# pola-rs/polars

Measured on NVIDIA H100. Metric: group_by_agg_rows_per_sec, higher is better.
Workload: dtype int64/float64

## Files before the change

### polars_b200/csrc/groupby.cu

```cuda
#include <algorithm>
#include <cmath>
#include <cstdio>
#include <cstdlib>

#include "common.cuh"
#include "dev_utils.cuh"
#include "groupby.h"
#include "groupby_dev.cuh"

namespace plb {

__device__ __forceinline__ uint64_t make_policy_evict_last() {
    uint64_t p; asm volatile("createpolicy.fractional.L2::evict_last.b64 %0, 1.0;" : "=l"(p)); return p;
}
__device__ __forceinline__ uint64_t tbl_load(const uint64_t* p, uint64_t pol, int hint) {
    uint64_t v;
    if (hint & 2) asm volatile("ld.global.ca.u64 %0, [%1];" : "=l"(v) : "l"(p) : "memory");
    else if (hint & 1) asm volatile("ld.global.cg.L2::cache_hint.u64 %0, [%1], %2;" : "=l"(v) : "l"(p), "l"(pol));
    else v = __ldcg(reinterpret_cast<const unsigned long long*>(p));
    return v;
}

__device__ __forceinline__ uint64_t* gb_resolve(const GbTableDev& T, uint64_t key, uint64_t slot, uint64_t k, uint64_t pol, int hint) {
    const uint64_t mask = T.cap - 1;
// ... 316 lines not shown
            __syncwarp();
        }
#pragma unroll
        for (int r = 0; r < 2; r++) {
            if (kind[r] < 0 || hidx[r] >= 0) continue;
            uint64_t* e = kind[r] == 0 ? gb_resolve(T, key[r], slot[r], k0[r], 0, khint) : gb_special(T, kind[r] - 1);
            if (e) gb_apply_row<MAXC>(L, T, B, e, 2 * p + r, [&](int c) { return raw[c][r]; });
        }
    }
    gb_tail_row(L, T, B);
    __syncwarp();
    for (int h = lane; h < H.rows; h += 32) {
        const uint64_t* arow = wacc + h * row_words;
        if ((uint32_t)arow[1] == 0) continue;
        gb_merge_row(L, T, arow, h == H.n_hot ? 1 : (h == H.n_hot + 1 ? 2 : 0));
    }
}

__global__ void k_gb_init(uint64_t* entries, int64_t n_entries, int stride, int soa, int pw, const __grid_constant__ GbLayout L) {
    const int64_t total = n_entries * stride;
    for (int64_t i = (int64_t)blockIdx.x * blockDim.x + threadIdx.x; i < total; i += (int64_t)gridDim.x * blockDim.x) {
        int w = soa ? (int)(i / n_entries) : (int)(i % stride);
        if (pw) {
            if (w == 1 || w == 2) w = ((i - n_entries) & 1) ? pw : 1;
            else if (w == pw) w = 2;
        }
        uint64_t v = 0;
        if (w == 0) v = GB_EMPTY; else if (w == 1) v = GB_W1_INIT; else if (w - 2 < L.n_words) v = L.init[w - 2];
        entries[i] = v;
    }
}

constexpr int GB_CAND_MAX = 1024;
struct GbSampleStats { unsigned distinct, f1, f2, adjacent, nulls, empties, n_cand, pad; };
struct GbCandidate { uint64_t key; uint64_t mult; };
__global__ void k_gb_estimate(const void* keys, const uint32_t* key_validity, int key_dtype, int64_t n, int64_t m, uint64_t* scratch, unsigned* mult, uint64_t cap, int shift, GbSampleStats* stats) {
    for (int64_t i = (int64_t)blockIdx.x * blockDim.x + threadIdx.x; i < m; i += (int64_t)gridDim.x * blockDim.x) {
        int64_t row = (int64_t)(((unsigned __int128)i * (unsigned __int128)n) / (unsigned __int128)m);
        bool ins = false, adj = false, isnull = false, isempty = false;
        if (key_validity == nullptr || bit_get(key_validity, row)) {
            uint64_t key = load_key_rt(keys, key_dtype, row);
            adj = row + 1 < n && load_key_rt(keys, key_dtype, row + 1) == key && (key_validity == nullptr || bit_get(key_validity, row + 1));
            if (key != GB_EMPTY) {
                uint64_t slot = table_hash(key) >> shift;
                for (int pr = 0; pr < (int)cap; pr++) {
                    uint64_t k = __ldcg(reinterpret_cast<const unsigned long long*>(scratch + slot));
                    if (k == GB_EMPTY) {
                        unsigned long long old = atomicCAS(reinterpret_cast<unsigned long long*>(scratch + slot), (unsigned long long)GB_EMPTY, (unsigned long long)key);
                        if (old == GB_EMPTY) { ins = true; k = key; } else k = old;
                    }
                    if (k == key) { atomicAdd(mult + slot, 1u); break; }
                    slot = (slot + 1) & (cap - 1);
                }
            } else isempty = true;
        } else {
            isnull = true;
            adj = row + 1 < n && !bit_get(key_validity, row + 1);
        }
        unsigned act = __activemask();
        unsigned b = __ballot_sync(act, ins), a = __ballot_sync(act, adj), bn = __ballot_sync(act, isnull), be = __ballot_sync(act, isempty);
        if (lane_id() == (unsigned)(__ffs(act) - 1)) {
            if (b) atomicAdd(&stats->distinct, (unsigned)__popc(b));
            if (a) atomicAdd(&stats->adjacent, (unsigned)__popc(a));
            if (bn) atomicAdd(&stats->nulls, (unsigned)__popc(bn));
            if (be) atomicAdd(&stats->empties, (unsigned)__popc(be));
        }
    }
}
__global__ void k_gb_estimate_stats(const uint64_t* scratch, const unsigned* mult, int64_t cap, unsigned hot_thr, GbSampleStats* stats, GbCandidate* cand) {
    unsigned f1 = 0, f2 = 0;
    for (int64_t i = (int64_t)blockIdx.x * blockDim.x + threadIdx.x; i < cap; i += (int64_t)gridDim.x * blockDim.x) {
        const unsigned c = mult[i];
        f1 += c == 1; f2 += c == 2;
        if (c >= hot_thr) {
            const unsigned at = atomicAdd(&stats->n_cand, 1u);
            if (at < GB_CAND_MAX) { cand[at].key = scratch[i]; cand[at].mult = c; }
        }
    }
    f1 = __reduce_add_sync(0xffffffffu, f1); f2 = __reduce_add_sync(0xffffffffu, f2);
    if (lane_id() == 0) { if (f1) atomicAdd(&stats->f1, f1); if (f2) atomicAdd(&stats->f2, f2); }
}
__global__ void k_fill_u64(uint64_t* p, uint64_t v, int64_t n) {
    for (int64_t i = (int64_t)blockIdx.x * blockDim.x + threadIdx.x; i < n; i += (int64_t)gridDim.x * blockDim.x) p[i] = v;
}

__device__ __forceinline__ void gb_merge_row(const GbLayout& L, const GbTableDev& T, const uint64_t* src, int meta, int64_t sws, int64_t sslot, int spw) {
    uint64_t* e = meta == 1 ? gb_special(T, 0) : (meta == 2 ? gb_special(T, 1) : gb_find_or_insert(T, src[0]));
    if (!e) return;
    const uint64_t lf = src[gb_woff(sslot, 1, sws, spw)];
    if ((uint32_t)lf) atomicAdd(reinterpret_cast<unsigned*>(gb_wp(T, e, 1)), (uint32_t)lf);
    if ((uint32_t)(lf >> 32) != 0xFFFFFFFFu) atomicMin(reinterpret_cast<unsigned*>(gb_wp(T, e, 1)) + 1, (uint32_t)(lf >> 32));
    for (int w = 0; w < L.n_words; w++) {
        const uint64_t v = src[gb_woff(sslot, 2 + w, sws, spw)];
        if (v == L.init[w]) continue;
        uint64_t* a = gb_wp(T, e, 2 + w);
        switch (L.slot_op[w]) {
            case W_ADD_F64: atomicAdd(reinterpret_cast<double*>(a), __longlong_as_double((long long)v)); break;
            case W_MIN_S64: atomicMin(reinterpret_cast<long long*>(a), (long long)v); break;
            case W_MAX_S64: atomicMax(reinterpret_cast<long long*>(a), (long long)v); break;
            case W_MIN_U64: case W_MIN_F64: atomicMin(reinterpret_cast<unsigned long long*>(a), (unsigned long long)v); break;
            case W_MAX_U64: case W_MAX_F64: atomicMax(reinterpret_cast<unsigned long long*>(a), (unsigned long long)v); break;
            default: atomicAdd(reinterpret_cast<unsigned long long*>(a), (unsigned long long)v); break;
        }
    }
}
__global__ void __launch_bounds__(256) k_gb_merge(const __grid_constant__ GbLayout L, const __grid_constant__ GbTableDev T, const uint64_t* __restrict__ rows, int64_t n_rows, int64_t src_es, int64_t src_ws, int table_mode, int64_t src_cap, int src_pw) {
    for (int64_t r = (int64_t)blockIdx.x * blockDim.x + threadIdx.x; r < n_rows; r += (int64_t)gridDim.x * blockDim.x) {
        const uint64_t* src = rows + r * src_es;
        int meta;
        if (table_mode) { if (src[0] == GB_EMPTY) continue; meta = r == src_cap ? 1 : (r == src_cap + 1 ? 2 : 0); }
        else meta = (int)src[(L.n_words + 2) * src_ws];
        gb_merge_row(L, T, src, meta, src_ws, r, table_mode ? src_pw : 0);
    }
// ... 391 lines not shown
    if (d >= m * 0.995) return n;
    double lo = d, hi = n > d ? n : d;
    for (int it = 0; it < 60; it++) { double G = 0.5 * (lo + hi); double ex = G * (1.0 - exp(-m / G)); if (ex < d) lo = G; else hi = G; }
    return hi;
}

void GroupByState::build_hot_list(const void* cand_v, int n_cand, bool null_hot, bool empty_hot, double m) {
    const GbCandidate* cand = static_cast<const GbCandidate*>(cand_v);
    hot = GbHotDev{}; hot_share = 0; hot_buf.reset();
    if (!knob_int("BL_K5_HOTKEYS", 1) || (n_cand <= 0 && !null_hot && !empty_hot)) return;
    std::vector<GbCandidate> c(cand, cand + std::max(n_cand, 0));
    std::sort(c.begin(), c.end(), [](const GbCandidate& a, const GbCandidate& b) { return a.mult > b.mult || (a.mult == b.mult && a.key < b.key); });
    const int row_words = 2 + L.n_words;
    int n_hot = std::min<int>((int)c.size(), std::min(GB_HOT_MAX, 512 / row_words - 2));
    if (n_hot < 0) n_hot = 0;
    if (!c.empty()) hot_share = (double)c[0].mult / m;
    std::vector<unsigned char> h(GB_HOT_SLOTS * 8 + GB_HOT_SLOTS, 0);
    uint64_t* hk = reinterpret_cast<uint64_t*>(h.data());
    unsigned char* hi = h.data() + GB_HOT_SLOTS * 8;
    for (int i = 0; i < GB_HOT_SLOTS; i++) hk[i] = GB_EMPTY;
    for (int i = 0; i < n_hot; i++) {
        unsigned sl = (unsigned)(table_hash(c[i].key) >> (64 - GB_HOT_BITS));
        while (hk[sl] != GB_EMPTY) sl = (sl + 1) & (GB_HOT_SLOTS - 1);
        hk[sl] = c[i].key; hi[sl] = (unsigned char)i;
    }
    hot_buf = dev_alloc(h.size());
    PLB_CUDA(cudaMemcpyAsync(hot_buf->p, h.data(), h.size(), cudaMemcpyHostToDevice, ctx().stream));
    PLB_CUDA(cudaStreamSynchronize(ctx().stream));
    hot.keys = as<uint64_t>(hot_buf); hot.idx = reinterpret_cast<const uint8_t*>(hot_buf->p) + GB_HOT_SLOTS * 8;
    hot.n_hot = n_hot; hot.null_hot = null_hot ? 1 : 0; hot.empty_hot = empty_hot ? 1 : 0; hot.rows = n_hot + 2;
}

uint64_t GroupByState::choose_cap(const DevCol& key, int64_t n_total) {
    double G, G_raw, G_upper = 0;
    if (expected_groups > 0) G = G_raw = (double)expected_groups;
    else {
        const int64_t n = key.len, m = std::min<int64_t>(n, 65536);
        const uint64_t scap = 1 << 18;
        const size_t tail_bytes = sizeof(GbSampleStats) + sizeof(GbCandidate) * GB_CAND_MAX;
        DevPtr scratch = dev_alloc(scap * 8), mult = dev_alloc(scap * 4 + tail_bytes);
        GbSampleStats* dstats = reinterpret_cast<GbSampleStats*>(as<unsigned>(mult) + scap);
        GbCandidate* dcand = reinterpret_cast<GbCandidate*>(dstats + 1);
        const double nt = (double)std::max<int64_t>(n_total, n);
        const double hot_knob = knob_double("BL_K5_HOT_ROWS", 30000.0), hot_rows = hot_knob >= 0 ? hot_knob : 30000.0;
        const unsigned hot_thr = (unsigned)std::max(12.0, std::ceil(hot_rows * (double)m / nt));
        PLB_LAUNCH("k5_fill", k_fill_u64, grid_for(scap, 256), 256, 0, as<uint64_t>(scratch), GB_EMPTY, (int64_t)scap);
        dev_memset(mult->p, 0, scap * 4 + sizeof(GbSampleStats));
        PLB_LAUNCH("k5_estimate", k_gb_estimate, grid_for(m, 256), 256, 0, key.v(), key.vm(), key.dtype, n, m, as<uint64_t>(scratch), as<unsigned>(mult), scap, 64 - 18, dstats);
        PLB_LAUNCH("k5_estimate", k_gb_estimate_stats, grid_for(scap, 256), 256, 0, as<uint64_t>(scratch), as<unsigned>(mult), (int64_t)scap, hot_thr, dstats, dcand);
        std::vector<unsigned char> hbuf(tail_bytes);
        PLB_CUDA(cudaMemcpyAsync(hbuf.data(), dstats, tail_bytes, cudaMemcpyDeviceToHost, ctx().stream));
        PLB_CUDA(cudaStreamSynchronize(ctx().stream));
        GbSampleStats st; memcpy(&st, hbuf.data(), sizeof st);
        const GbCandidate* cand = reinterpret_cast<const GbCandidate*>(hbuf.data() + sizeof(GbSampleStats));
        G_raw = estimate_groups((double)st.distinct, (double)m, nt);
        if (m < n && st.f1 > 0) {
            const double chao = (double)st.distinct + (double)st.f1 * ((double)st.f1 - 1.0) / (2.0 * ((double)st.f2 + 1.0));
            if (chao > G_raw) G_raw = chao;
            if ((double)st.distinct >= (double)m * 0.995 && st.f2 >= 16) G_raw = std::min(G_raw, 2.0 * chao);
        }
        sample_adjacent = m > 0 ? (double)st.adjacent / (double)m : 0.0;
        if (m < n && sample_adjacent > 0.5) {
            const double q = 1.0 - sample_adjacent;
            const double runs = nt * std::min(1.0, q + 3.0 * std::sqrt(q * sample_adjacent / (double)m) + 2.0 / (double)m) + 1.0;
            if (runs < G_raw) G_raw = runs;
        }
        G = G_raw * 1.25 + 64;
        if (G > nt) G = nt;
        if (G_raw > nt) G_raw = nt;
        G_upper = std::min(nt, (double)st.distinct + (double)st.f1 / (double)m * nt);
        build_hot_list(cand, (int)std::min<unsigned>(st.n_cand, GB_CAND_MAX), st.nulls >= hot_thr, st.empties >= hot_thr, (double)m);
    }
    est_groups = (int64_t)(G_raw * 1.25) + 2;
    const double lf_knob = knob_double("BL_K5_LF", 60.0) / 100.0, lf = (lf_knob > 0.05 && lf_knob < 0.95) ? lf_knob : 0.6;
    uint64_t c = pow2_at_least(G / lf);
    const double l2_budget = 0.55 * (double)ctx().l2_bytes;
    if ((double)c * L.stride * 8 > l2_budget && G_raw / ((double)c / 2) <= 0.8 && c > 1024) c >>= 1;
    while (G_upper / lf > (double)c && (double)(2 * c) * L.stride * 8 <= l2_budget) c <<= 1;
    if (getenv("BL_K5_DEBUG"))
        fprintf(stderr, "[k5] rows=%lld est_groups=%.0f upper=%.0f cap=%llu (%.1f MB) hot_keys=%d null_hot=%d empty_hot=%d hot_share=%.4f adjacent=%.3f\n", (long long)n_total, G_raw, G_upper,
                (unsigned long long)c, (double)c * L.stride * 8 / 1e6, hot.n_hot, hot.null_hot, hot.empty_hot, hot_share, sample_adjacent);
    return c;
}

template <int KEY_ELEM, int KEY_CANON, bool KEY_NULLS, int PAIRS, bool BULK>
static void launch_consume_p(const GbLayout& L, const GbTableDev& T, const GbBatch& B, int grid) {
    with_at_least<1, 2, 4, 8>(L.n_cols, [&](auto maxc) {
        constexpr int MAXC = decltype(maxc)::value, P = MAXC == 8 ? 1 : PAIRS;
        const size_t smem = BULK ? (size_t)2 * P * 256 * 16 : 0;
        PLB_LAUNCH("k5_groupby_agg", (k_gb_consume<KEY_ELEM, KEY_CANON, KEY_NULLS, MAXC, P, BULK>), grid, 256, smem, L, T, B);
    });
}
template <int KEY_ELEM, int KEY_CANON, bool KEY_NULLS>
static void launch_consume(const GbLayout& L, const GbTableDev& T, const GbBatch& B, int grid) {
    const int pairs = knob_int("BL_K5_PAIRS", 1) == 2 ? 2 : 1;
    if (T.pw && T.bulk_lanes > 0 && L.pair_k >= 0) {
        bool lean = KEY_ELEM == 8 && KEY_CANON == 0 && T.bulk_lanes == 32 && !T.hint && !L.need_first && L.need_len && L.n_cols >= 1 && L.n_cols <= 3 &&
                    knob_int("BL_K5_LEAN", 1) != 0;
        bool nulls = KEY_NULLS;
        for (int c = 0; lean && c < L.n_cols; c++) { lean = B.cols[c].elem == 8 && L.col_kbegin[c + 1] - L.col_kbegin[c] <= 2; nulls = nulls || B.cols[c].validity != nullptr; }
        if (lean) with_at_least<1, 2, 3>(L.n_cols, [&](auto nc) { with_bool(nulls, [&](auto nl) {
            PLB_LAUNCH("k5_groupby_agg", (k_gb_consume_lean<decltype(nc)::value, decltype(nl)::value>), grid, 256, (size_t)2 * 256 * 16, L, T, B);
        }); });
        else launch_consume_p<KEY_ELEM, KEY_CANON, KEY_NULLS, 1, true>(L, T, B, grid);
    }
    else if (pairs == 2) launch_consume_p<KEY_ELEM, KEY_CANON, KEY_NULLS, 2, false>(L, T, B, grid);
// ... 529 lines not shown
```

### polars_b200/csrc/groupby.h

```cpp
#pragma once
#include <cstdlib>
#include <type_traits>

#include "common.cuh"

namespace plb {

inline int knob_int(const char* name, int dflt) { const char* e = getenv(name); return e ? atoi(e) : dflt; }
inline double knob_double(const char* name, double dflt) { const char* e = getenv(name); return e ? atof(e) : dflt; }

template <int V> using IntC = std::integral_constant<int, V>;
template <class F> void with_key_form(int key_dtype, F&& f) {
    if (dtype_size(key_dtype) == 8) { if (key_dtype == BL_FLOAT64) f(IntC<8>{}, IntC<1>{}); else f(IntC<8>{}, IntC<0>{}); }
    else { if (key_dtype == BL_FLOAT32) f(IntC<4>{}, IntC<2>{}); else f(IntC<4>{}, IntC<0>{}); }
}
template <int V, int... Vs, class F> void with_at_least(int n, F&& f) {
    if constexpr (sizeof...(Vs) == 0) f(IntC<V>{});
    else if (n <= V) f(IntC<V>{});
    else with_at_least<Vs...>(n, f);
}
template <class F> void with_bool(bool b, F&& f) { if (b) f(std::true_type{}); else f(std::false_type{}); }

constexpr uint64_t GB_EMPTY = 0x8000000000000000ULL;
constexpr uint64_t GB_W1_INIT = 0xFFFFFFFF00000000ULL;
// ... 22 lines not shown
    }
    return (int64_t)w * ws;
}
struct GbBatch {
    const void* keys; const uint32_t* key_validity; int64_t n; uint32_t row_base; int32_t key_dtype;
    GbColDev cols[GB_MAX_COLS];
};


constexpr int GB_HOT_MAX = 62;
constexpr int GB_HOT_BITS = 8;
constexpr int GB_HOT_SLOTS = 1 << GB_HOT_BITS;
struct GbHotDev { const uint64_t* keys; const uint8_t* idx; int32_t n_hot, null_hot, empty_hot, rows; };

struct GbDense { DevPtr keys, first, len, words, ctl; int64_t Gb = 0; bool ready = false; };

struct AggPlan { int kind, in_dtype, out_dtype; int main, nullcnt; bool nullable; };

struct GroupByState {
    int key_dtype;
    std::vector<int> agg_kinds, agg_dtypes;
    int64_t expected_groups;
    std::vector<AggPlan> plans;
    GbLayout L;
    bool lean_shape = false;
    int pair_word = 0;
    GbTableDev T{};
    DevPtr entries, status;
    uint64_t cap = 0;
    int64_t rows_seen = 0;
    int64_t merged_rows = 0;
    int64_t est_groups = 0;
    double sample_adjacent = 0;
    GbHotDev hot{};
    double hot_share = 0;
    DevPtr hot_buf;

    GroupByState(int key_dt, const std::vector<int>& kinds, const std::vector<int>& dtypes, const std::vector<int>& nullable, int64_t expected, bool track_first);
    void consume_all(const DevCol& key, const std::vector<const DevCol*>& values);
    bool consume_radix(const DevCol& key, const std::vector<const DevCol*>& values, uint64_t planned_cap);
    GbDense dense;
    void consume_pipelined(const DevCol& key, const std::vector<const DevCol*>& values, int64_t chunk_rows, const std::vector<cudaEvent_t>& ready);
    void consume(const DevCol& key, const std::vector<const DevCol*>& values, int64_t row_base);
    void merge_partials(const uint64_t* rows, int64_t n_rows);
    void merge_partial_regions(const uint64_t* const* ptrs, const int64_t* counts, int n_regions);
    DevPtr export_partials(int n_partitions, int* row_words_out, int64_t* offsets_host);
    void export_partials_p2p(int n_ranks, int my_rank, void* const* windows, int64_t rows_per_src, int* row_words_out, int64_t* sent_rows);
    void export_partials_p2p_async(int n_ranks, int my_rank, void* const* window_halves, int64_t rows_per_src, uint64_t epoch, int* row_words_out);
    void merge_window_async(const void* own_half, int n_ranks, int64_t rows_per_src, uint64_t epoch);
    void settle();
    int read_status();
    bool defer_status = false;
    const DevCol* redo_key = nullptr; std::vector<const DevCol*> redo_values; uint64_t redo_cap = 0;
    void finish(bool maintain_order, const DevCol* key_col_for_gather, DevCol& out_key, std::vector<DevCol>& out_aggs, DevCol* out_first = nullptr);
    void reset();
    int64_t count_groups();

   private:
    void alloc_table(uint64_t new_cap);
    int smem_table_cap() const;
    bool bind_columns(const DevCol& key, const std::vector<const DevCol*>& values, int64_t row_base, int pw, int max_cols, GbBatch& B, GbLayout& Lb) const;
    void note_batch_shape(const DevCol& key, const std::vector<const DevCol*>& values);
    uint64_t choose_cap(const DevCol& key, int64_t n_total);
    void build_hot_list(const void* candidates, int n_cand, bool null_hot, bool empty_hot, double sample_rows);
    void launch_batch(const DevCol& key, const std::vector<const DevCol*>& values, int64_t row_base);
    void grow(uint64_t new_cap);
// ... 4 lines not shown
```

### polars_b200/csrc/groupby_radix.cu

```cuda
#include <algorithm>
#include <cstdlib>

#include "common.cuh"
#include "dev_utils.cuh"
#include "groupby.h"
#include "groupby_dev.cuh"

namespace plb {

constexpr int GBR_THREADS = 512;
constexpr int GBR_MAX_LOGB = 13;
constexpr int GBR_NCW = 31, GBR_NCT = GBR_NCW * 32;

struct GbRadixDev {
    uint64_t* recs;
    const unsigned long long* off;
    unsigned* cursor;
    unsigned* counts;
    int logB, roww;
    uint64_t* special;
    int* status;
};

template <int KEY_ELEM> __device__ __forceinline__ void gbr_load_pair(const void* col, int64_t r0, int64_t n, uint64_t& a, uint64_t& b) {
    a = 0; b = 0;
    if (r0 + 1 < n) gb_load_pair<KEY_ELEM>(col, r0, a, b);
    else if (r0 < n) a = KEY_ELEM == 8 ? reinterpret_cast<const uint64_t*>(col)[r0] : reinterpret_cast<const uint32_t*>(col)[r0];
}
__device__ __forceinline__ void gbr_load_pair_rt(const void* col, int elem, int64_t r0, int64_t n, uint64_t& a, uint64_t& b) {
    if (elem == 8) gbr_load_pair<8>(col, r0, n, a, b); else gbr_load_pair<4>(col, r0, n, a, b);
}

template <int KEY_ELEM, int KEY_CANON>
__global__ void __launch_bounds__(512) k_gbr_hist(const void* __restrict__ keys, int64_t n, int logB, unsigned* __restrict__ counts) {
    extern __shared__ unsigned h_s[];
    const int B = 1 << logB;
    for (int i = threadIdx.x; i < B; i += blockDim.x) h_s[i] = 0;
    __syncthreads();
    const int64_t npairs = (n + 1) >> 1;
    for (int64_t p = (int64_t)blockIdx.x * blockDim.x + threadIdx.x; p < npairs; p += (int64_t)gridDim.x * blockDim.x) {
        uint64_t k0, k1;
        gbr_load_pair<KEY_ELEM>(keys, 2 * p, n, k0, k1);
        k0 = canon_key<KEY_CANON>(k0); k1 = canon_key<KEY_CANON>(k1);
        if (k0 != GB_EMPTY) atomicAdd(&h_s[(unsigned)(table_hash(k0) >> (64 - logB))], 1u);
        if (2 * p + 1 < n && k1 != GB_EMPTY) atomicAdd(&h_s[(unsigned)(table_hash(k1) >> (64 - logB))], 1u);
    }
    __syncthreads();
    for (int i = threadIdx.x; i < B; i += blockDim.x) if (h_s[i]) atomicAdd(&counts[i], h_s[i]);
}
__global__ void __launch_bounds__(1024) k_gbr_offsets(const unsigned* __restrict__ counts, int B, unsigned long long pad_units, unsigned pad_each, unsigned align,
                                                      unsigned long long* __restrict__ off, unsigned* __restrict__ cursor) {
    __shared__ unsigned long long wsum[32];
    __shared__ unsigned long long carry_s;
    if (threadIdx.x == 0) carry_s = 0;
    __syncthreads();
    const unsigned lane = lane_id(), warp = threadIdx.x >> 5;
    for (int base = 0; base < B; base += 1024) {
        const int i = base + threadIdx.x;
        unsigned long long c = 0;
        if (i < B) { c = counts[i]; c += (c < pad_units ? c : pad_units) * pad_each; c = (c + align - 1) & ~(unsigned long long)(align - 1); cursor[i] = 0; }
        unsigned long long x = c;
        for (int o = 1; o < 32; o <<= 1) { const unsigned long long y = __shfl_up_sync(0xffffffffu, x, o); if (lane >= (unsigned)o) x += y; }
        if (lane == 31) wsum[warp] = x;
        __syncthreads();
        if (warp == 0) {
            unsigned long long s = wsum[lane], t = s;
            for (int o = 1; o < 32; o <<= 1) { const unsigned long long y = __shfl_up_sync(0xffffffffu, t, o); if (lane >= (unsigned)o) t += y; }
            wsum[lane] = t - s;
        }
        __syncthreads();
        const unsigned long long incl = carry_s + wsum[warp] + x;
        if (i < B) off[i] = incl - c;
        __syncthreads();
        if (threadIdx.x == 1023) carry_s = incl;
        __syncthreads();
    }
    if (threadIdx.x == 0) off[B] = carry_s;
}

__device__ __forceinline__ void gbr_apply_special(const GbLayout& L, const GbBatch& Bt, uint64_t* sp, const uint64_t* raw) {
    atomicAdd(reinterpret_cast<unsigned long long*>(sp), 1ull);
    for (int c = 0; c < L.n_cols; c++)
        for (int k = L.col_kbegin[c]; k < L.col_kbegin[c + 1]; k++) {
            uint64_t* a = sp + 1 + L.wslot[k];
            const int dt = Bt.cols[c].dtype;
            switch (L.wop[k]) {
                case W_ADD_INT: atomicAdd(reinterpret_cast<unsigned long long*>(a), (unsigned long long)raw_to_int(dt, raw[c])); break;
                case W_ADD_F64: atomicAdd(reinterpret_cast<double*>(a), raw_to_f64(dt, raw[c])); break;
                case W_MIN_S64: atomicMin(reinterpret_cast<long long*>(a), (long long)raw_to_int(dt, raw[c])); break;
                case W_MAX_S64: atomicMax(reinterpret_cast<long long*>(a), (long long)raw_to_int(dt, raw[c])); break;
                case W_MIN_U64: atomicMin(reinterpret_cast<unsigned long long*>(a), (unsigned long long)raw[c]); break;
                case W_MAX_U64: atomicMax(reinterpret_cast<unsigned long long*>(a), (unsigned long long)raw[c]); break;
                case W_MIN_F64: { const double f = raw_to_f64(dt, raw[c]); if (f == f) atomicMin(reinterpret_cast<unsigned long long*>(a), (unsigned long long)f64_to_ordered(f)); break; }
// ... 25 lines not shown
        uint64_t k[RPT]; unsigned pk[RPT];
#pragma unroll
        for (int j = 0; j < RPT / 2; j++) gbr_load_pair<KEY_ELEM>(Bt.keys, base + 2 * (int64_t)(j * THREADS + tid), n, k[2 * j], k[2 * j + 1]);
#pragma unroll
        for (int j = 0; j < RPT; j++) {
            const int64_t r = base + 2 * (int64_t)((j >> 1) * THREADS + tid) + (j & 1);
            pk[j] = 0xFFFFFFFFu;
            if (r < n) {
                k[j] = canon_key<KEY_CANON>(k[j]);
                if (k[j] == GB_EMPTY) pk[j] = 0xFFFFFFFEu;
                else { const unsigned b = (unsigned)(table_hash(k[j]) >> (64 - logB)); pk[j] = (b << 16) | atomicAdd(&hist[b], 1u); }
            }
        }
        __syncthreads();
        const int bins = (B + THREADS - 1) / THREADS;
        unsigned mine = 0;
        for (int q = 0; q < bins; q++) { const int p = tid * bins + q; if (p < B) { unsigned c = hist[p]; if (BULK) c = (c + 1u) & ~1u; mine += c; } }
        unsigned x = mine;
        for (int o = 1; o < 32; o <<= 1) { const unsigned y = __shfl_up_sync(0xffffffffu, x, o); if (lane >= o) x += y; }
        if (lane == 31) warp_tot[warp] = x;
        __syncthreads();
        if (warp == 0) {
            unsigned w = lane < THREADS / 32 ? warp_tot[lane] : 0, s = w;
            for (int o = 1; o < 32; o <<= 1) { const unsigned y = __shfl_up_sync(0xffffffffu, s, o); if (lane >= o) s += y; }
            if (lane < THREADS / 32) warp_tot[lane] = s - w;
        }
        __syncthreads();
        unsigned run = warp_tot[warp] + x - mine;
        for (int q = 0; q < bins; q++) {
            const int p = tid * bins + q;
            if (p < B) {
                const unsigned c = hist[p], cp = BULK ? ((c + 1u) & ~1u) : c;
                start[p] = run;
                gpos[p] = cp ? atomicAdd(&R.cursor[p], cp) : 0u;
                run += cp;
            }
        }
        if (BULK) bulk_wait_read0();
        __syncthreads();
        if (BULK) for (int p = tid; p < B; p += THREADS) { const unsigned c = hist[p]; if (c & 1u) { uint64_t* pad = stage + (size_t)(start[p] + c) * ROWW; pad[0] = GB_EMPTY;
#pragma unroll
                                                                                                      for (int w = 1; w < ROWW; w++) pad[w] = 0; } }
#pragma unroll
        for (int j = 0; j < RPT / 2; j++) {
            const int64_t r0 = base + 2 * (int64_t)(j * THREADS + tid);
            uint64_t v[NC > 0 ? NC : 1][2];
#pragma unroll
            for (int c = 0; c < NC; c++) gbr_load_pair_rt(Bt.cols[c].values, Bt.cols[c].elem, r0, n, v[c][0], v[c][1]);
#pragma unroll
            for (int e = 0; e < 2; e++) {
                const unsigned q = pk[2 * j + e];
                if (q == 0xFFFFFFFFu) continue;
                if (q == 0xFFFFFFFEu) {
                    uint64_t raw[NC > 0 ? NC : 1];
#pragma unroll
                    for (int c = 0; c < NC; c++) raw[c] = v[c][e];
                    gbr_apply_special(L, Bt, R.special, raw);
                    continue;
                }
                const unsigned bkt = q >> 16, pos = start[bkt] + (q & 0xFFFFu);
                uint64_t* rec = stage + (size_t)pos * ROWW;
                rec[0] = k[2 * j + e];
#pragma unroll
                for (int c = 0; c < NC; c++) rec[1 + c] = v[c][e];
                if (!BULK) sp[pos] = (uint16_t)bkt;
            }
        }
        if (BULK) fence_async_smem();
        __syncthreads();
        if (BULK) {
            for (int p = tid; p < B; p += THREADS) {
                const unsigned c = hist[p], cp = (c + 1u) & ~1u;
                if (cp) bulk_s2g(R.recs + (R.off[p] + gpos[p]) * ROWW, stage + (size_t)start[p] * ROWW, cp * ROWW * 8);
            }
            bulk_commit();
        } else {
            const unsigned total = start[B - 1] + hist[B - 1];
            for (unsigned w = tid; w < total * ROWW; w += THREADS) {
                const unsigned row = w / ROWW, c = w - row * ROWW;
                const unsigned p = sp[row];
                R.recs[(R.off[p] + gpos[p] + (row - start[p])) * ROWW + c] = stage[w];
            }
            __syncthreads();
        }
    }
    if (BULK) bulk_wait0();
}

constexpr int GBR_WC_THREADS = 256, GBR_WC_F = 4;
template <int ROWW> constexpr int gbr_wc_rpt() { return ROWW <= 3 ? 8 : 4; }
template <int ROWW, int KEY_ELEM, int RPT>
__device__ __forceinline__ void gbr_wc_load(const GbBatch& Bt, int64_t base, uint64_t (&k)[RPT], uint64_t (&v)[ROWW > 1 ? ROWW - 1 : 1][RPT]) {
#pragma unroll
    for (int j = 0; j < RPT / 2; j++) {
        const int64_t r0 = base + 2 * (int64_t)(j * GBR_WC_THREADS + threadIdx.x);
        gbr_load_pair<KEY_ELEM>(Bt.keys, r0, Bt.n, k[2 * j], k[2 * j + 1]);
#pragma unroll
        for (int c = 0; c < ROWW - 1; c++) gbr_load_pair_rt(Bt.cols[c].values, Bt.cols[c].elem, r0, Bt.n, v[c][2 * j], v[c][2 * j + 1]);
    }
}

template <int ROWW, int KEY_ELEM, int KEY_CANON>
__global__ void __launch_bounds__(GBR_WC_THREADS, 2) k_gbr_scatter_wc(const __grid_constant__ GbLayout L, const __grid_constant__ GbBatch Bt, const __grid_constant__ GbRadixDev R) {
    constexpr int THREADS = GBR_WC_THREADS, F = GBR_WC_F, RPT = gbr_wc_rpt<ROWW>(), T = THREADS * RPT, NC = ROWW - 1, NCX = NC > 0 ? NC : 1, CH = F * ROWW;
    constexpr unsigned NONE = 0xFFFFFFFFu;
    const int logB = R.logB, B = 1 << logB, tid = threadIdx.x;
    extern __shared__ __align__(16) uint64_t gbr_smem[];
    uint64_t* buf = gbr_smem;
    unsigned* fill = reinterpret_cast<unsigned*>(buf + (size_t)B * CH);
    const int64_t n = Bt.n, ntiles = (n + T - 1) / T;
    for (int p = tid; p < B; p += THREADS) fill[p] = 0;
    uint64_t k[RPT], v[NCX][RPT], kn[RPT], vn[NCX][RPT];
    if ((int64_t)blockIdx.x < ntiles) gbr_wc_load<ROWW, KEY_ELEM, RPT>(Bt, (int64_t)blockIdx.x * T, kn, vn);
    for (int64_t tile = blockIdx.x; tile < ntiles; tile += gridDim.x) {
// ... 23 lines not shown
#pragma unroll
        for (int e = 0; e < RPT; e++)
            if (pk[e] != NONE) { const unsigned s = atomicAdd(&fill[pk[e] >> 16], 1u); pk[e] |= s; last = max(last, s / F); }
        bulk_wait_read0();
        __syncthreads();
        for (unsigned r = 0;; r++) {
#pragma unroll
            for (int e = 0; e < RPT; e++) {
                const unsigned s = pk[e] & 0xFFFFu;
                if (pk[e] == NONE || s / F != r) continue;
                uint64_t* rec = buf + (size_t)(pk[e] >> 16) * CH + (s % F) * ROWW;
                rec[0] = k[e];
#pragma unroll
                for (int c = 0; c < NC; c++) rec[1 + c] = v[c][e];
            }
            fence_async_smem();
            const bool more = __syncthreads_or(last > r);
            const unsigned full = (r + 1) * F;
            for (int p0 = 0; p0 < B; p0 += 4 * THREADS) {
                unsigned g[4];
#pragma unroll
                for (int q = 0; q < 4; q++) {
                    const int p = p0 + q * THREADS + tid;
                    g[q] = NONE;
                    if (p < B) {
                        const unsigned f = fill[p];
                        if (f >= full) g[q] = atomicAdd(&R.cursor[p], (unsigned)F);
                        if (!more) fill[p] = f % F;
                    }
                }
#pragma unroll
                for (int q = 0; q < 4; q++) {
                    const int p = p0 + q * THREADS + tid;
                    if (g[q] != NONE) bulk_s2g(R.recs + (R.off[p] + g[q]) * ROWW, buf + (size_t)p * CH, CH * 8);
                }
            }
            bulk_commit();
            if (!more) break;
            bulk_wait_read0();
            __syncthreads();
        }
    }
    __syncthreads();
    for (int p = tid; p < B; p += THREADS) {
        const unsigned f = fill[p];
        if (f == 0) continue;
        for (unsigned i = f; i < F; i++) buf[(size_t)p * CH + i * ROWW] = GB_EMPTY;
        fence_async_smem();
        const unsigned g = atomicAdd(&R.cursor[p], (unsigned)F);
        bulk_s2g(R.recs + (R.off[p] + g) * ROWW, buf + (size_t)p * CH, CH * 8);
    }
    bulk_commit();
    bulk_wait0();
}

struct GbDenseDev { uint64_t* keys; uint32_t* first; uint32_t* len; uint64_t* words; int64_t Gb; unsigned long long* cursor; };

constexpr int GBR_NST = 2;
template <int ROWW>
__global__ void __launch_bounds__(1024) k_gbr_agg(const __grid_constant__ GbLayout L, const __grid_constant__ GbBatch Bt, const __grid_constant__ GbRadixDev R, const __grid_constant__ GbDenseDev D, unsigned S) {
    constexpr int NST = GBR_NST, CR = GBR_NCT, NC = ROWW - 1;
    extern __shared__ __align__(128) uint64_t gbr_smem2[];
    uint64_t* ring = gbr_smem2;
    uint64_t* tkey = ring + (size_t)NST * CR * ROWW;
    uint64_t* tacc = tkey + S;
    unsigned* tlen = reinterpret_cast<unsigned*>(tacc + (size_t)L.n_words * S);
    __shared__ uint64_t full[NST], empty[NST];
    __shared__ unsigned s_used, s_base;
    const int tid = threadIdx.x, warp = tid >> 5, lane = tid & 31, B = 1 << R.logB;
    if (tid == 0) { for (int s = 0; s < NST; s++) { mbar_init(&full[s], 1); mbar_init(&empty[s], GBR_NCW); } mbar_fence_init(); }
    __syncthreads();
    if (warp == GBR_NCW) {
        if (lane == 0) {
            unsigned q = 0;
            for (int p = blockIdx.x; p < B; p += gridDim.x) {
                const int64_t rows = (int64_t)R.cursor[p];
                const uint64_t* src = R.recs + R.off[p] * ROWW;
                const int nch = (int)((rows + CR - 1) / CR);
                for (int c = 0; c < nch; c++, q++) {
                    const int st = q % NST; const unsigned use = q / NST;
                    if (use > 0) while (!mbar_try_wait(&empty[st], (use - 1) & 1u)) {}
                    const int64_t crow = min((int64_t)CR, rows - (int64_t)c * CR);
                    const unsigned bytes = (unsigned)(((crow + 1) & ~(int64_t)1) * ROWW * 8);
                    mbar_expect_tx(&full[st], bytes);
                    bulk_g2s(ring + (size_t)st * CR * ROWW, src + (size_t)c * CR * ROWW, bytes, &full[st]);
                }
            }
        }
        return;
    }
    const unsigned max_used = S - (S >> 2);
    unsigned q = 0;
    for (int p = blockIdx.x; p < B; p += gridDim.x) {
        for (unsigned i = tid; i < S; i += GBR_NCT) { tkey[i] = GB_EMPTY; tlen[i] = 0; for (int w = 0; w < L.n_words; w++) tacc[(size_t)w * S + i] = L.init[w]; }
        if (tid == 0) s_used = 0;
        named_bar_sync(1, GBR_NCT);
        const int64_t rows = (int64_t)R.cursor[p];
        const int nch = (int)((rows + CR - 1) / CR);
        for (int c = 0; c < nch; c++, q++) {
            const int st = q % NST; const unsigned par = (q / NST) & 1u;
            while (!mbar_try_wait(&full[st], par)) {}
            const uint64_t* buf = ring + (size_t)st * CR * ROWW;
// ... 106 lines not shown
    if (!bind_columns(key, values, 0, 0, 4, Bt, Lb)) return false;
    const int roww = 1 + Lb.n_cols;
    const int64_t n = key.len;
    const size_t entry = 8 + 4 + 8 * (size_t)L.n_words;
    const size_t ring2 = (size_t)GBR_NST * GBR_NCT * roww * 8;
    unsigned S = 0; int logB = 6;
    for (const size_t total_kb : {(size_t)110, (size_t)222}) {
        if (total_kb * 1024 < ring2 + 1024 + 512 * entry) continue;
        S = (unsigned)((total_kb * 1024 - ring2 - 1024) / entry) & ~31u;
        const double per_bucket = 0.55 * (double)S;
        logB = 6;
        while (logB < GBR_MAX_LOGB && (double)est_groups / (double)(1 << logB) > per_bucket) logB++;
        if ((double)est_groups / (double)(1 << logB) <= 0.7 * (double)S) break;
        S = 0;
    }
    if (S == 0) return false;
    if (mode == 1) {
        const double l2_budget = 0.55 * (double)ctx().l2_bytes;
        if ((double)planned_cap * L.stride * 8 <= 2.0 * l2_budget) return false;
    }
    const int B = 1 << logB;
    int smem_optin = 0;
    PLB_CUDA(cudaDeviceGetAttribute(&smem_optin, cudaDevAttrMaxSharedMemoryPerBlockOptin, ctx().device));
    const bool wc_fits = gbr_wc_smem(B, roww) <= (size_t)smem_optin;
    const int store = knob_int("BL_K5R_STORE", 0);
    bool bulk = logB <= 9, wc = !bulk && wc_fits;
    if (store == 1 && gbr_scatter_smem(B, roww, false) <= (size_t)smem_optin) bulk = wc = false;
    else if (store == 2 && wc_fits) { bulk = false; wc = true; }
    else if (store == 3 && gbr_scatter_smem(B, roww, true) <= (size_t)smem_optin) { bulk = true; wc = false; }
    const int64_t ntiles = (n + GBR_THREADS * GBR_RPT - 1) / (GBR_THREADS * GBR_RPT);
    auto with_scatter_form = [&](auto f) { with_key_form(key.dtype, [&](auto e, auto c) { with_at_least<1, 2, 3, 4, 5>(roww, [&](auto w) { f(e, c, w); }); }); };
    int wc_grid = 0;
    if (wc) with_scatter_form([&](auto e, auto c, auto w) { wc_grid = scatter_wc_grid<decltype(w)::value, decltype(e)::value, decltype(c)::value>(B); });
    const int64_t pad_rows = bulk ? std::min<int64_t>(n, (int64_t)B * ntiles) : wc ? std::min<int64_t>(n, (int64_t)B * wc_grid) * (GBR_WC_F - 1) : 0;
    const int64_t rec_rows = n + pad_rows + (wc ? GBR_WC_F : 2) * (int64_t)B + 16;
    DevPtr recs, ctl;
    try {
        recs = dev_alloc((size_t)rec_rows * roww * 8);
        ctl = dev_alloc((size_t)B * 4 * 2 + (size_t)(B + 1) * 8 + (size_t)(1 + GB_MAX_WORDS) * 8 + 64);
    } catch (const Error&) { cudaGetLastError(); return false; }
    GbRadixDev R; memset(&R, 0, sizeof R);
    R.recs = as<uint64_t>(recs); R.logB = logB; R.roww = roww; R.status = as<int>(status);
    char* cp = reinterpret_cast<char*>(ctl->p);
    R.off = reinterpret_cast<unsigned long long*>(cp); cp += (size_t)(B + 1) * 8;
    R.special = reinterpret_cast<uint64_t*>(cp); cp += (size_t)(1 + GB_MAX_WORDS) * 8;
    R.counts = reinterpret_cast<unsigned*>(cp); cp += (size_t)B * 4;
    R.cursor = reinterpret_cast<unsigned*>(cp);
    dev_memset(ctl->p, 0, ctl->bytes);
    {
        uint64_t h[1 + GB_MAX_WORDS]; h[0] = 0; for (int w = 0; w < L.n_words; w++) h[1 + w] = L.init[w];
        PLB_CUDA(cudaMemcpyAsync(R.special, h, (size_t)(1 + L.n_words) * 8, cudaMemcpyHostToDevice, ctx().stream));
        PLB_CUDA(cudaStreamSynchronize(ctx().stream));
    }
    dev_memset(status->p, 0, 4);
    with_key_form(key.dtype, [&](auto e, auto c) {
        PLB_LAUNCH("k5r_histogram", (k_gbr_hist<decltype(e)::value, decltype(c)::value>), ctx().sm_count * 4, 512, (size_t)B * 4, key.v(), n, logB, R.counts);
    });
    if (wc) PLB_LAUNCH("k5r_offsets", k_gbr_offsets, 1, 1024, 0, R.counts, B, (unsigned long long)wc_grid, (unsigned)(GBR_WC_F - 1), (unsigned)GBR_WC_F, const_cast<unsigned long long*>(R.off), R.cursor);
    else PLB_LAUNCH("k5r_offsets", k_gbr_offsets, 1, 1024, 0, R.counts, B, (unsigned long long)ntiles, bulk ? 1u : 0u, 2u, const_cast<unsigned long long*>(R.off), R.cursor);
    with_scatter_form([&](auto e, auto c, auto w) {
        constexpr int E = decltype(e)::value, C = decltype(c)::value, ROWW = decltype(w)::value;
        if (wc) PLB_LAUNCH("k5r_scatter", (k_gbr_scatter_wc<ROWW, E, C>), wc_grid, GBR_WC_THREADS, gbr_wc_smem(B, ROWW), Lb, Bt, R);
        else launch_scatter<ROWW, E, C>(Lb, Bt, R, bulk);
    });
    const int64_t Gb = std::max<int64_t>(1024, std::min<int64_t>(n + 1, 3 * est_groups + (1 << 16)));
    dense.keys = dev_alloc((size_t)Gb * 8); dense.first = dev_alloc((size_t)Gb * 4); dense.len = dev_alloc((size_t)Gb * 4);
    dense.words = dev_alloc((size_t)Gb * 8 * std::max(L.n_words, 1)); dense.ctl = dev_alloc(16); dense.Gb = Gb;
    const long long ctl_init[2] = {0, -1};
    PLB_CUDA(cudaMemcpyAsync(dense.ctl->p, ctl_init, 16, cudaMemcpyHostToDevice, ctx().stream));
    GbDenseDev D{as<uint64_t>(dense.keys), as<uint32_t>(dense.first), as<uint32_t>(dense.len), as<uint64_t>(dense.words), Gb, as<unsigned long long>(dense.ctl)};
    with_at_least<1, 2, 3, 4, 5>(roww, [&](auto w) { launch_agg<decltype(w)::value>(Lb, Bt, R, D, S); });
    PLB_LAUNCH("k5r_special", k_gbr_append_special, 1, 32, 0, R.special, L.n_words, D, as<int>(status));
    const int st = read_scalar(as<int>(status));
    if (getenv("BL_K5_DEBUG")) fprintf(stderr, "[k5r] rows=%lld est_groups=%lld buckets=%d slots=%u bulk=%d store=%s status=%d\n", (long long)n, (long long)est_groups, B, S, (int)bulk,
                                      bulk ? "runs" : wc ? "wc" : "coalesced", st);
    if (st != 0) { dense = GbDense{}; dev_memset(status->p, 0, 4); return false; }
    dense.ready = true;
    rows_seen = n;
    return true;
}

}
```

Measured before the change: 26.80 billion.

## Skip radix histogram pass by sizing buckets from sampled frequency moments

The sampling kernel now also accumulates the second frequency moment (sum of c*(c-1)), which is used to estimate the variance of per-bucket row counts. When the estimated margin is small, each radix bucket gets a fixed capacity of mean plus five standard deviations, so the full histogram pass over the keys is skipped. Scatter kernels check the per-bucket cap and set an overflow status, in which case the whole pipeline reruns with the exact histogram. The setup kernel also initializes status and special rows on the device, replacing a host memcpy plus stream sync. The tradeoff is a larger allocation and a full rerun whenever the estimate is wrong.

```diff
diff --git a/polars_b200/csrc/groupby.cu b/polars_b200/csrc/groupby.cu
--- a/polars_b200/csrc/groupby.cu
+++ b/polars_b200/csrc/groupby.cu
@@ -372,7 +372,7 @@
 }
 
 constexpr int GB_CAND_MAX = 1024;
-struct GbSampleStats { unsigned distinct, f1, f2, adjacent, nulls, empties, n_cand, pad; };
+struct GbSampleStats { unsigned distinct, f1, f2, adjacent, nulls, empties, n_cand, pad; unsigned long long pairs; };
 struct GbCandidate { uint64_t key; uint64_t mult; };
 __global__ void k_gb_estimate(const void* keys, const uint32_t* key_validity, int key_dtype, int64_t n, int64_t m, uint64_t* scratch, unsigned* mult, uint64_t cap, int shift, GbSampleStats* stats) {
     for (int64_t i = (int64_t)blockIdx.x * blockDim.x + threadIdx.x; i < m; i += (int64_t)gridDim.x * blockDim.x) {
@@ -409,16 +409,19 @@
 }
 __global__ void k_gb_estimate_stats(const uint64_t* scratch, const unsigned* mult, int64_t cap, unsigned hot_thr, GbSampleStats* stats, GbCandidate* cand) {
     unsigned f1 = 0, f2 = 0;
+    unsigned long long pairs = 0;
     for (int64_t i = (int64_t)blockIdx.x * blockDim.x + threadIdx.x; i < cap; i += (int64_t)gridDim.x * blockDim.x) {
         const unsigned c = mult[i];
         f1 += c == 1; f2 += c == 2;
+        if (c > 1) pairs += (unsigned long long)c * (c - 1);
         if (c >= hot_thr) {
             const unsigned at = atomicAdd(&stats->n_cand, 1u);
             if (at < GB_CAND_MAX) { cand[at].key = scratch[i]; cand[at].mult = c; }
         }
     }
     f1 = __reduce_add_sync(0xffffffffu, f1); f2 = __reduce_add_sync(0xffffffffu, f2);
-    if (lane_id() == 0) { if (f1) atomicAdd(&stats->f1, f1); if (f2) atomicAdd(&stats->f2, f2); }
+    for (int o = 16; o > 0; o >>= 1) pairs += __shfl_xor_sync(0xffffffffu, pairs, o);
+    if (lane_id() == 0) { if (f1) atomicAdd(&stats->f1, f1); if (f2) atomicAdd(&stats->f2, f2); if (pairs) atomicAdd(&stats->pairs, pairs); }
 }
 __global__ void k_fill_u64(uint64_t* p, uint64_t v, int64_t n) {
     for (int64_t i = (int64_t)blockIdx.x * blockDim.x + threadIdx.x; i < n; i += (int64_t)gridDim.x * blockDim.x) p[i] = v;
@@ -876,7 +879,7 @@
 }
 
 uint64_t GroupByState::choose_cap(const DevCol& key, int64_t n_total) {
-    double G, G_raw, G_upper = 0;
+    double G, G_raw, G_upper = 0, f2 = 0;
     if (expected_groups > 0) G = G_raw = (double)expected_groups;
     else {
         const int64_t n = key.len, m = std::min<int64_t>(n, 65536);
@@ -913,9 +916,11 @@
         if (G > nt) G = nt;
         if (G_raw > nt) G_raw = nt;
         G_upper = std::min(nt, (double)st.distinct + (double)st.f1 / (double)m * nt);
+        if (m > 0) { const double q = (double)m / (double)n; f2 = (double)n + (double)st.pairs / (q * q); }
         build_hot_list(cand, (int)std::min<unsigned>(st.n_cand, GB_CAND_MAX), st.nulls >= hot_thr, st.empties >= hot_thr, (double)m);
     }
     est_groups = (int64_t)(G_raw * 1.25) + 2;
+    est_f2 = f2 > 0 ? std::max(f2, (double)key.len * (double)key.len / (double)est_groups) : 0.0;
     const double lf_knob = knob_double("BL_K5_LF", 60.0) / 100.0, lf = (lf_knob > 0.05 && lf_knob < 0.95) ? lf_knob : 0.6;
     uint64_t c = pow2_at_least(G / lf);
     const double l2_budget = 0.55 * (double)ctx().l2_bytes;
diff --git a/polars_b200/csrc/groupby.h b/polars_b200/csrc/groupby.h
--- a/polars_b200/csrc/groupby.h
+++ b/polars_b200/csrc/groupby.h
@@ -78,6 +78,7 @@
     int64_t merged_rows = 0;
     int64_t est_groups = 0;
     double sample_adjacent = 0;
+    double est_f2 = 0;
     GbHotDev hot{};
     double hot_share = 0;
     DevPtr hot_buf;
diff --git a/polars_b200/csrc/groupby_radix.cu b/polars_b200/csrc/groupby_radix.cu
--- a/polars_b200/csrc/groupby_radix.cu
+++ b/polars_b200/csrc/groupby_radix.cu
@@ -11,6 +11,7 @@
 constexpr int GBR_THREADS = 512;
 constexpr int GBR_MAX_LOGB = 13;
 constexpr int GBR_NCW = 31, GBR_NCT = GBR_NCW * 32;
+constexpr unsigned GBR_NO_ROOM = 0xFFFFFFFFu;
 
 struct GbRadixDev {
     uint64_t* recs;
@@ -19,6 +20,7 @@
     unsigned* counts;
     int logB, roww;
     uint64_t* special;
+    unsigned cap;
     int* status;
 };
 
@@ -48,17 +50,22 @@
     __syncthreads();
     for (int i = threadIdx.x; i < B; i += blockDim.x) if (h_s[i]) atomicAdd(&counts[i], h_s[i]);
 }
-__global__ void __launch_bounds__(1024) k_gbr_offsets(const unsigned* __restrict__ counts, int B, unsigned long long pad_units, unsigned pad_each, unsigned align,
-                                                      unsigned long long* __restrict__ off, unsigned* __restrict__ cursor) {
+__host__ __device__ __forceinline__ unsigned long long gbr_stream_records(unsigned long long rows, unsigned long long pad_units, unsigned pad_each, unsigned align) {
+    rows += (rows < pad_units ? rows : pad_units) * pad_each;
+    return (rows + align - 1) & ~(unsigned long long)(align - 1);
+}
+__global__ void __launch_bounds__(1024) k_gbr_offsets(const __grid_constant__ GbLayout L, const unsigned* __restrict__ counts, unsigned long long rows, int B, unsigned long long pad_units,
+                                                      unsigned pad_each, unsigned align, unsigned long long* __restrict__ off, unsigned* __restrict__ cursor, uint64_t* __restrict__ special, int* __restrict__ status) {
     __shared__ unsigned long long wsum[32];
     __shared__ unsigned long long carry_s;
-    if (threadIdx.x == 0) carry_s = 0;
+    if (threadIdx.x == 0) { carry_s = 0; *status = 0; special[0] = 0; }
+    if (threadIdx.x < (unsigned)L.n_words) special[1 + threadIdx.x] = L.init[threadIdx.x];
     __syncthreads();
     const unsigned lane = lane_id(), warp = threadIdx.x >> 5;
     for (int base = 0; base < B; base += 1024) {
         const int i = base + threadIdx.x;
         unsigned long long c = 0;
-        if (i < B) { c = counts[i]; c += (c < pad_units ? c : pad_units) * pad_each; c = (c + align - 1) & ~(unsigned long long)(align - 1); cursor[i] = 0; }
+        if (i < B) { c = gbr_stream_records(counts ? counts[i] : rows, pad_units, pad_each, align); cursor[i] = 0; }
         unsigned long long x = c;
         for (int o = 1; o < 32; o <<= 1) { const unsigned long long y = __shfl_up_sync(0xffffffffu, x, o); if (lane >= (unsigned)o) x += y; }
         if (lane == 31) wsum[warp] = x;
@@ -150,7 +157,9 @@
             if (p < B) {
                 const unsigned c = hist[p], cp = BULK ? ((c + 1u) & ~1u) : c;
                 start[p] = run;
-                gpos[p] = cp ? atomicAdd(&R.cursor[p], cp) : 0u;
+                unsigned g = cp ? atomicAdd(&R.cursor[p], cp) : 0u;
+                if (g + cp > R.cap) { *R.status = 2; g = GBR_NO_ROOM; }
+                gpos[p] = g;
                 run += cp;
             }
         }
@@ -189,15 +198,15 @@
         if (BULK) {
             for (int p = tid; p < B; p += THREADS) {
                 const unsigned c = hist[p], cp = (c + 1u) & ~1u;
-                if (cp) bulk_s2g(R.recs + (R.off[p] + gpos[p]) * ROWW, stage + (size_t)start[p] * ROWW, cp * ROWW * 8);
+                if (cp && gpos[p] != GBR_NO_ROOM) bulk_s2g(R.recs + (R.off[p] + gpos[p]) * ROWW, stage + (size_t)start[p] * ROWW, cp * ROWW * 8);
             }
             bulk_commit();
         } else {
             const unsigned total = start[B - 1] + hist[B - 1];
             for (unsigned w = tid; w < total * ROWW; w += THREADS) {
                 const unsigned row = w / ROWW, c = w - row * ROWW;
-                const unsigned p = sp[row];
-                R.recs[(R.off[p] + gpos[p] + (row - start[p])) * ROWW + c] = stage[w];
+                const unsigned p = sp[row], g = gpos[p];
+                if (g != GBR_NO_ROOM) R.recs[(R.off[p] + g + (row - start[p])) * ROWW + c] = stage[w];
             }
             __syncthreads();
         }
@@ -287,7 +296,9 @@
 #pragma unroll
                 for (int q = 0; q < 4; q++) {
                     const int p = p0 + q * THREADS + tid;
-                    if (g[q] != NONE) bulk_s2g(R.recs + (R.off[p] + g[q]) * ROWW, buf + (size_t)p * CH, CH * 8);
+                    if (g[q] == NONE) continue;
+                    if (g[q] + F <= R.cap) bulk_s2g(R.recs + (R.off[p] + g[q]) * ROWW, buf + (size_t)p * CH, CH * 8);
+                    else *R.status = 2;
                 }
             }
             bulk_commit();
@@ -303,7 +314,8 @@
         for (unsigned i = f; i < F; i++) buf[(size_t)p * CH + i * ROWW] = GB_EMPTY;
         fence_async_smem();
         const unsigned g = atomicAdd(&R.cursor[p], (unsigned)F);
-        bulk_s2g(R.recs + (R.off[p] + g) * ROWW, buf + (size_t)p * CH, CH * 8);
+        if (g + F <= R.cap) bulk_s2g(R.recs + (R.off[p] + g) * ROWW, buf + (size_t)p * CH, CH * 8);
+        else *R.status = 2;
     }
     bulk_commit();
     bulk_wait0();
@@ -323,6 +335,7 @@
     __shared__ uint64_t full[NST], empty[NST];
     __shared__ unsigned s_used, s_base;
     const int tid = threadIdx.x, warp = tid >> 5, lane = tid & 31, B = 1 << R.logB;
+    if (*R.status == 2) return;
     if (tid == 0) { for (int s = 0; s < NST; s++) { mbar_init(&full[s], 1); mbar_init(&empty[s], GBR_NCW); } mbar_fence_init(); }
     __syncthreads();
     if (warp == GBR_NCW) {
@@ -495,8 +508,12 @@
     auto with_scatter_form = [&](auto f) { with_key_form(key.dtype, [&](auto e, auto c) { with_at_least<1, 2, 3, 4, 5>(roww, [&](auto w) { f(e, c, w); }); }); };
     int wc_grid = 0;
     if (wc) with_scatter_form([&](auto e, auto c, auto w) { wc_grid = scatter_wc_grid<decltype(w)::value, decltype(e)::value, decltype(c)::value>(B); });
-    const int64_t pad_rows = bulk ? std::min<int64_t>(n, (int64_t)B * ntiles) : wc ? std::min<int64_t>(n, (int64_t)B * wc_grid) * (GBR_WC_F - 1) : 0;
-    const int64_t rec_rows = n + pad_rows + (wc ? GBR_WC_F : 2) * (int64_t)B + 16;
+    const unsigned long long pad_units = wc ? (unsigned long long)wc_grid : (unsigned long long)ntiles;
+    const unsigned pad_each = wc ? GBR_WC_F - 1 : bulk ? 1u : 0u, align = wc ? GBR_WC_F : 2u;
+    const double mean = (double)n / B, margin = 5.0 * std::sqrt(est_f2 / B);
+    unsigned long long bucket_rows = est_f2 > 0 && margin <= 0.5 * mean ? (unsigned long long)std::ceil(mean + margin) : 0;
+    const int64_t exact_rows = n + std::min<int64_t>(n, (int64_t)B * (int64_t)pad_units) * pad_each + (int64_t)align * B + 16;
+    int64_t rec_rows = bucket_rows ? (int64_t)B * (int64_t)gbr_stream_records(bucket_rows, pad_units, pad_each, align) + 16 : exact_rows;
     DevPtr recs, ctl;
     try {
         recs = dev_alloc((size_t)rec_rows * roww * 8);
@@ -509,38 +526,47 @@
     R.special = reinterpret_cast<uint64_t*>(cp); cp += (size_t)(1 + GB_MAX_WORDS) * 8;
     R.counts = reinterpret_cast<unsigned*>(cp); cp += (size_t)B * 4;
     R.cursor = reinterpret_cast<unsigned*>(cp);
-    dev_memset(ctl->p, 0, ctl->bytes);
-    {
-        uint64_t h[1 + GB_MAX_WORDS]; h[0] = 0; for (int w = 0; w < L.n_words; w++) h[1 + w] = L.init[w];
-        PLB_CUDA(cudaMemcpyAsync(R.special, h, (size_t)(1 + L.n_words) * 8, cudaMemcpyHostToDevice, ctx().stream));
-        PLB_CUDA(cudaStreamSynchronize(ctx().stream));
-    }
-    dev_memset(status->p, 0, 4);
-    with_key_form(key.dtype, [&](auto e, auto c) {
-        PLB_LAUNCH("k5r_histogram", (k_gbr_hist<decltype(e)::value, decltype(c)::value>), ctx().sm_count * 4, 512, (size_t)B * 4, key.v(), n, logB, R.counts);
-    });
-    if (wc) PLB_LAUNCH("k5r_offsets", k_gbr_offsets, 1, 1024, 0, R.counts, B, (unsigned long long)wc_grid, (unsigned)(GBR_WC_F - 1), (unsigned)GBR_WC_F, const_cast<unsigned long long*>(R.off), R.cursor);
-    else PLB_LAUNCH("k5r_offsets", k_gbr_offsets, 1, 1024, 0, R.counts, B, (unsigned long long)ntiles, bulk ? 1u : 0u, 2u, const_cast<unsigned long long*>(R.off), R.cursor);
-    with_scatter_form([&](auto e, auto c, auto w) {
-        constexpr int E = decltype(e)::value, C = decltype(c)::value, ROWW = decltype(w)::value;
-        if (wc) PLB_LAUNCH("k5r_scatter", (k_gbr_scatter_wc<ROWW, E, C>), wc_grid, GBR_WC_THREADS, gbr_wc_smem(B, ROWW), Lb, Bt, R);
-        else launch_scatter<ROWW, E, C>(Lb, Bt, R, bulk);
-    });
     const int64_t Gb = std::max<int64_t>(1024, std::min<int64_t>(n + 1, 3 * est_groups + (1 << 16)));
     dense.keys = dev_alloc((size_t)Gb * 8); dense.first = dev_alloc((size_t)Gb * 4); dense.len = dev_alloc((size_t)Gb * 4);
     dense.words = dev_alloc((size_t)Gb * 8 * std::max(L.n_words, 1)); dense.ctl = dev_alloc(16); dense.Gb = Gb;
-    const long long ctl_init[2] = {0, -1};
-    PLB_CUDA(cudaMemcpyAsync(dense.ctl->p, ctl_init, 16, cudaMemcpyHostToDevice, ctx().stream));
     GbDenseDev D{as<uint64_t>(dense.keys), as<uint32_t>(dense.first), as<uint32_t>(dense.len), as<uint64_t>(dense.words), Gb, as<unsigned long long>(dense.ctl)};
-    with_at_least<1, 2, 3, 4, 5>(roww, [&](auto w) { launch_agg<decltype(w)::value>(Lb, Bt, R, D, S); });
-    PLB_LAUNCH("k5r_special", k_gbr_append_special, 1, 32, 0, R.special, L.n_words, D, as<int>(status));
-    const int st = read_scalar(as<int>(status));
-    if (getenv("BL_K5_DEBUG")) fprintf(stderr, "[k5r] rows=%lld est_groups=%lld buckets=%d slots=%u bulk=%d store=%s status=%d\n", (long long)n, (long long)est_groups, B, S, (int)bulk,
-                                      bulk ? "runs" : wc ? "wc" : "coalesced", st);
-    if (st != 0) { dense = GbDense{}; dev_memset(status->p, 0, 4); return false; }
-    dense.ready = true;
-    rows_seen = n;
-    return true;
-}
-
-}
+    for (;;) {
+        const unsigned long long cap = bucket_rows ? gbr_stream_records(bucket_rows, pad_units, pad_each, align) : 0;
+        R.cap = cap ? (unsigned)cap : ~0u;
+        if (!bucket_rows) {
+            dev_memset(R.counts, 0, (size_t)B * 4);
+            with_key_form(key.dtype, [&](auto e, auto c) {
+                PLB_LAUNCH("k5r_histogram", (k_gbr_hist<decltype(e)::value, decltype(c)::value>), ctx().sm_count * 4, 512, (size_t)B * 4, key.v(), n, logB, R.counts);
+            });
+        }
+        PLB_LAUNCH("k5r_setup", k_gbr_offsets, 1, 1024, 0, L, bucket_rows ? nullptr : R.counts, bucket_rows, B, pad_units, pad_each, align,
+                   const_cast<unsigned long long*>(R.off), R.cursor, R.special, R.status);
+        with_scatter_form([&](auto e, auto c, auto w) {
+            constexpr int E = decltype(e)::value, C = decltype(c)::value, ROWW = decltype(w)::value;
+            if (wc) PLB_LAUNCH("k5r_scatter", (k_gbr_scatter_wc<ROWW, E, C>), wc_grid, GBR_WC_THREADS, gbr_wc_smem(B, ROWW), Lb, Bt, R);
+            else launch_scatter<ROWW, E, C>(Lb, Bt, R, bulk);
+        });
+        dev_memset(dense.ctl->p, 0, 8); dev_memset(static_cast<char*>(dense.ctl->p) + 8, 0xFF, 8);
+        with_at_least<1, 2, 3, 4, 5>(roww, [&](auto w) { launch_agg<decltype(w)::value>(Lb, Bt, R, D, S); });
+        PLB_LAUNCH("k5r_special", k_gbr_append_special, 1, 32, 0, R.special, L.n_words, D, as<int>(status));
+        const int st = read_scalar(as<int>(status));
+        if (getenv("BL_K5_DEBUG"))
+            fprintf(stderr, "[k5r] rows=%lld est_groups=%lld buckets=%d slots=%u bulk=%d store=%s sizing=%s cap=%llu status=%d\n", (long long)n, (long long)est_groups, B, S, (int)bulk,
+                    bulk ? "runs" : wc ? "wc" : "coalesced", bucket_rows ? "sample" : "exact", cap, st);
+        if (st == 2 && bucket_rows) {
+            bucket_rows = 0;
+            if (exact_rows > rec_rows) {
+                recs.reset();
+                try { recs = dev_alloc((size_t)exact_rows * roww * 8); } catch (const Error&) { cudaGetLastError(); dense = GbDense{}; dev_memset(status->p, 0, 4); return false; }
+                R.recs = as<uint64_t>(recs); rec_rows = exact_rows;
+            }
+            continue;
+        }
+        if (st != 0) { dense = GbDense{}; dev_memset(status->p, 0, 4); return false; }
+        dense.ready = true;
+        rows_seen = n;
+        return true;
+    }
+}
+
+}
```

After: 28.69 billion, median of 6. +7.0%, better.
